# fhgyuanshen/HybridGL

Measured on AMD Instinct MI355X. Metric: images/sec (whole node), higher is better.
Workload: dtype f32 via fp16x3 split MFMA (fp32 accumulate)

## Files before the change

hybridgl_amd/_lib.py:

```python
import ctypes as C
import os

_HERE = os.path.dirname(os.path.abspath(__file__))
LIB_PATH = os.path.join(_HERE, "libhybridgl.so")

c_float_p = C.POINTER(C.c_float)
c_u8_p = C.POINTER(C.c_uint8)
c_i32_p = C.POINTER(C.c_int32)
c_i64_p = C.POINTER(C.c_int64)


class HybridGLError(RuntimeError):
    pass


class HglSentence(C.Structure):
    _fields_ = [("sentence_row", C.c_int), ("noun_phrase_row", C.c_int), ("other_row0", C.c_int), ("n_other", C.c_int),
                ("dirflag", C.c_int), ("relaword", C.c_int), ("has_other_nouns", C.c_int), ("black", C.c_float),
                ("imgattn", C.c_void_p), ("target", C.c_void_p)]


class HglGroupRef(C.Structure):
    _fields_ = [("hybrid", C.c_void_p), ("text", C.c_void_p), ("T", C.c_int), ("boxes", C.c_void_p), ("masks", C.c_void_p),
                ("N", C.c_int), ("H", C.c_int), ("W", C.c_int), ("sentences", C.POINTER(HglSentence)), ("S", C.c_int),
# ... 123 lines not shown
    "hgl_resize_bilinear_aa": (_I, [_VP, _I, _I, _I, _VP, _I, _I, _VP]),
    "hgl_resize_bilinear": (_I, [_VP, _I, _I, _I, _VP, _I, _I, _VP]),
    "hgl_mask_resize": (_I, [_VP, _I, _I, _I, _I, _VP, _VP]),
    "hgl_calculate_score": (_I, [_VP, _VP, _I, _I, _I, _F, _VP, _VP]),
    "hgl_coherence_workspace_bytes": (_SZ, [_I, _I, _I]),
    "hgl_coherence_scores": (_I, [_VP, _VP, _I, _I, _I, _I, _F, _VP, _VP, _SZ, _VP]),
    "hgl_iou": (_I, [_VP, _VP, _LL, _VP, _VP]),
    "hgl_iou_select": (_I, [_VP, _VP, _I, _VP, _LL, _VP, _VP]),
    "hgl_score_sentence_workspace_bytes": (_SZ, [_I, _I]),
    "hgl_score_sentence": (_I, [_VP, _VP, _VP, _VP, _I, _F, _VP, _VP, _I, _I, _F, _I, _I, _F, _I, _I,
                                _VP, _VP, _VP, _VP, _SZ, _VP]),
    "hgl_synthesize_views": (_I, [_VP, _VP, _VP, _VP, _I, _I, _I, _I, _VP, _VP, _VP]),
    "hgl_resize_pil_bilinear_workspace_bytes": (_SZ, [_I, _I, _I]),
    "hgl_resize_pil_bilinear": (_I, [_VP, _I, _I, _I, _I, _I, _VP, _VP, _I, _VP, _VP, _I, _VP, _VP, _SZ, _VP]),
    "hgl_sam_encode_workspace_bytes": (_SZ, [C.POINTER(HglSamEncoderW)]),
    "hgl_sam_encode": (_I, [C.POINTER(HglSamEncoderW), _VP, _I, _I, _VP, _VP, _SZ, _VP]),
    "hgl_sam_encode_batch_workspace_bytes": (_SZ, [C.POINTER(HglSamEncoderW), _I]),
    "hgl_sam_encode_batch": (_I, [C.POINTER(HglSamEncoderW), C.POINTER(C.c_void_p), C.POINTER(C.c_int), C.POINTER(C.c_int), _I,
                                  _VP, _VP, _SZ, _VP]),
    "hgl_sam_relpos_tables_workspace_bytes": (_SZ, [_I, _I, _I, _I]),
    "hgl_sam_relpos_tables": (_I, [_VP, _VP, _VP, _I, _I, _I, _I, _I, _I, _VP, _VP, _VP, _VP, _VP, _SZ, _VP]),
    "hgl_sam_dense_pe": (_I, [C.POINTER(HglSamDecoderW), _VP, _VP, _VP]),
    "hgl_sam_decode_workspace_bytes": (_SZ, [C.POINTER(HglSamDecoderW), _I]),
    "hgl_sam_decode_points": (_I, [C.POINTER(HglSamDecoderW), _VP, _VP, _I, _VP, _VP, _VP, _SZ, _VP]),
    "hgl_sam_decode_points_gated": (_I, [C.POINTER(HglSamDecoderW), _VP, _VP, _I, C.c_float, _VP, _VP, _VP, _SZ, _VP]),
    "hgl_sam_decode_multi_workspace_bytes": (_SZ, [C.POINTER(HglSamDecoderW), _I, _I]),
    "hgl_sam_decode_points_multi": (_I, [C.POINTER(HglSamDecoderW), _VP, _VP, _I, _I, _VP, _VP, _VP, _SZ, _VP]),
    "hgl_sam_decode_points_multi_gated": (_I, [C.POINTER(HglSamDecoderW), _VP, _VP, _I, _I, C.c_float, _VP, _VP, _VP, _SZ, _VP]),
    "hgl_sam_decode_prompts": (_I, [C.POINTER(HglSamDecoderW), _VP, _VP, _VP, _I, _VP, _I, _I, _VP, _VP, _VP, _SZ, _VP]),
    "hgl_sam_embed_masks": (_I, [C.POINTER(HglSamDecoderW), _VP, _I, _VP, _VP]),
    "hgl_sam_decoder_fusion": (_I, [_I]),
    "hgl_attention_presplit": (_I, [_I]),
    "hgl_attention_presplit_f32": (_I, [_VP, _I, _I, _I, _I, _I, _VP, _I, C.c_float, _I, _VP, _I, _I, _VP, C.c_size_t, _VP]),
    "hgl_sam_postprocess_workspace_bytes": (_SZ, [_I]),
    "hgl_sam_postprocess": (_I, [_VP, _VP, _I, _I, _I, _I, _I, _I, _I, _I, _F, _F, _F, _F, _VP, _VP, _VP, _VP, _VP,
                                 _VP, _SZ, _VP]),
    "hgl_nms": (_I, [_VP, _VP, _VP, _I, _F, _VP, _VP, _VP]),
    "hgl_nms_segments": (_I, [_VP, _VP, _VP, _VP, _I, _I, _F, _VP, _VP, _VP]),
    "hgl_nms_large_workspace_bytes": (_SZ, [_I]),
    "hgl_nms_large": (_I, [_VP, _VP, _VP, _I, _F, _VP, _VP, _VP, _SZ, _VP]),
    "hgl_box_near_crop_edge": (_I, [_VP, _I, C.POINTER(C.c_int32), C.POINTER(C.c_int32), _F, _VP, _VP]),
    "hgl_remove_small_regions_workspace_bytes": (_SZ, [_I, _I, _I]),
    "hgl_remove_small_regions": (_I, [_VP, _I, _I, _I, _I, _I, _VP, _VP, _VP, _SZ, _VP]),
    "hgl_remove_small_regions_boxes": (_I, [_VP, _I, _I, _I, _I, _I, _VP, _VP, _VP, _VP, _SZ, _VP]),
    "hgl_mask_boxes": (_I, [_VP, _I, _I, _I, _VP, _VP]),
    "hgl_gather_masks": (_I, [_VP, _VP, _VP, _I, _LL, _VP, _VP]),
    "hgl_gen_dir_mask": (_I, [_I, _I, _I, _VP, _VP]),
    "hgl_relation_boxes": (_I, [_VP, _VP, _VP, _VP, _I, _I, _VP, _VP]),
    "hgl_gaussian_blur_u8_workspace_bytes": (_SZ, [_I, _I, _I]),
    "hgl_gaussian_blur_u8": (_I, [_VP, _I, _I, _I, C.POINTER(C.c_double), _I, _VP, _VP, _SZ, _VP]),
    "hgl_cv_gaussian_kernel_q8": (_I, [_I, C.c_double, C.POINTER(C.c_uint16)]),
    "hgl_gaussian_blur_u8_q8": (_I, [_VP, _I, _I, _I, C.POINTER(C.c_uint16), C.POINTER(C.c_uint16), _I, _VP, _VP, _SZ, _VP]),
    "hgl_score_ref_workspace_bytes": (_SZ, [_I, _I, _I, _I, _I]),
    "hgl_score_ref": (_I, [_VP, _VP, _I, _VP, _VP, _I, _I, _I, _I, C.POINTER(HglSentence), _I, C.c_float, C.c_float, _I, _I, C.c_float,
                           _VP, _VP, _VP, _VP, _VP, _VP, _VP, _SZ, _VP]),
    "hgl_score_group_workspace_bytes": (_SZ, [C.POINTER(HglGroupRef), _I, _I]),
    "hgl_score_group": (_I, [C.POINTER(HglGroupRef), _I, _I, C.c_float, C.c_float, C.c_float, _VP, _VP, _SZ, _VP]),
    "hgl_score_group_sweep_workspace_bytes": (_SZ, [C.POINTER(HglGroupRef), _I, _I, C.POINTER(HglSweepConfig), _I]),
    "hgl_score_group_sweep": (_I, [C.POINTER(HglGroupRef), C.POINTER(HglSweepRef), _I, _I, C.c_float, C.POINTER(HglSweepConfig), _I,
                                   _VP, _VP, _VP, _SZ, _VP]),
    "hgl_u8_to_chw_lut": (_I, [_VP, _I, _I, _I, _VP, _VP, _VP]),
    "hgl_gt_mask_from_polygons": (_I, [_VP, _VP, _I, _I, _I, _VP, _VP]),
    "hgl_gt_mask_from_rle_counts": (_I, [_VP, _I, _I, _I, _VP, _VP]),
    "hgl_gt_mask_from_rle_string": (_I, [C.c_char_p, _I, _I, _VP, _VP]),
    "hgl_rle_encode_mask": (_I, [_VP, _I, _I, _VP, _LL, C.POINTER(C.c_longlong)]),
    "hgl_rle_to_string": (_I, [_VP, _LL, C.c_char_p, _SZ, C.POINTER(C.c_size_t)]),
# ... 56 lines not shown
```

hybridgl_amd/csrc/attention_ps.hip:

```cpp
#include "hgl_common.h"
#include "attn_tile.h"
#include <stdlib.h>
#include <mutex>
#include <type_traits>

namespace {

typedef __attribute__((address_space(3))) void lds_void_t;

constexpr int PS_CHUNK = 32;

enum { PS_PLAIN = 0, PS_WIN14 = 1, PS_RELT = 2 };

struct PsArgs {
  const _Float16 *hi, *lo;
  int ld, qcol, kcol, vcol;
  long long sb;
  int B, H, S;
  float* out;
  _Float16 *out_hi, *out_lo;
  int ldo;
  long long sob;
  float scale;
  int mask_kind;
  const uint8_t* keep;
  int keep_b0, keep_n;
  const float *rel_h, *rel_w;
  int kh, kw;
  const _Float16 *tabh_hi, *tabh_lo, *tabw_hi, *tabw_lo;
  int nqb;
  int dbg;
};
#ifdef HGL_DIAG
#define PS_DBG(a) ((a).dbg)
#else
#define PS_DBG(a) 0
#endif

__device__ __forceinline__ void ps_glds16(const void* sbase, unsigned voff, unsigned lds_addr) {
  unsigned keep;
  asm volatile("s_mov_b32 %0, m0\n\ts_mov_b32 m0, %3\n\ts_nop 0\n\tglobal_load_lds_dwordx4 %1, %2\n\ts_mov_b32 m0, %0"
               : "=&s"(keep)
               : "v"(voff), "s"(sbase), "s"(lds_addr)
               : "memory");
}
// ... 204 lines not shown
  const auto sw = __builtin_amdgcn_permlane32_swap(u, u, false, false);
  return fmaxf(__builtin_bit_cast(float, (unsigned)sw[0]), __builtin_bit_cast(float, (unsigned)sw[1]));
}
__device__ __forceinline__ float ps_add_halves(float x) {
  const unsigned u = __builtin_bit_cast(unsigned, x);
  const auto sw = __builtin_amdgcn_permlane32_swap(u, u, false, false);
  return __builtin_bit_cast(float, (unsigned)sw[0]) + __builtin_bit_cast(float, (unsigned)sw[1]);
}
template <int HD>
struct PspGeom {
  static constexpr int KS = HD / 16, DT = (HD + 31) / 32;
  static constexpr int KSL = HD / 4 + 1, KP = KSL * 8;
  static constexpr int VSL = 12, VP = VSL * 8;
  static constexpr int NIK = (PS_CHUNK * KSL + 63) / 64;
  static constexpr int NJK = (NIK + 3) / 4;
  static constexpr int KSTAGE = NIK * 1024;
  static constexpr int NIV = 2 * PS_CHUNK * VSL / 64;
  static constexpr int NJV = NIV / 4;
  static constexpr int VSTAGE = NIV * 1024;
  static constexpr int VL_OFF = PS_CHUNK * VSL * 16;
  static constexpr int K_RING = 0, V_RING = 3 * KSTAGE, E_OFF = V_RING + 2 * VSTAGE;
  static_assert(DT * 32 <= VP && NIV % 4 == 0, "geometry");
};
constexpr int PSP_EBYTES = PS_EROWS * 64;

template <int HD, int MODE>
constexpr size_t psp_lds_bytes() {
  return (size_t)PspGeom<HD>::E_OFF + (MODE == PS_WIN14 ? PSP_EBYTES : 0) + 256;
}

template <int HD, int MODE, int QT = 1>
__global__ __launch_bounds__(256, 2) void attn_psp_kernel(PsArgs a, const unsigned char* __restrict__ etab) {
  static_assert(QT == 1 || (QT == 2 && MODE == PS_PLAIN), "two query tiles per wave: the plain mode only");
  using G = PspGeom<HD>;
  constexpr int KS = G::KS, DT = G::DT, KP = G::KP, VP = G::VP;
  extern __shared__ __attribute__((aligned(1024))) unsigned char ps_smem[];
  uint8_t* const keepL = ps_smem + G::E_OFF + (MODE == PS_WIN14 ? PSP_EBYTES : 0);

  const int t = threadIdx.x, lane = t & 63;
  const int wave = __builtin_amdgcn_readfirstlane(t >> 6);
  const int r = lane & 31, h = lane >> 5;
  const float NEG_INF = __int_as_float(NEG_BIG_BITS);
  constexpr float LOG2E = 1.4426950408889634f;
  const float sl2e = a.scale * LOG2E;
  const float inv_scale = 1.0f / a.scale;
  const float rescale_thr = 5.5f * inv_scale;

  const unsigned ldb = (unsigned)a.ld * 2u;
  const unsigned lo_delta = (unsigned)((const char*)a.lo - (const char*)a.hi);
  const unsigned vrel = (unsigned)(a.vcol - a.kcol) * 2u;
  unsigned k_row[G::NJK], k_col[G::NJK], v_row[G::NJV], v_col[G::NJV];
#pragma unroll
  for (int j = 0; j < G::NJK; ++j) {
    const unsigned n = 64u * (unsigned)(wave + 4 * j) + (unsigned)lane;
    unsigned row = n / (unsigned)G::KSL;
    const unsigned c = n - row * (unsigned)G::KSL;
    unsigned col = 0;
    if (c < (unsigned)(HD / 8)) col = 16u * c;
    else if (c < (unsigned)(HD / 4)) col = 16u * (c - (unsigned)(HD / 8)) + lo_delta;
    if (row >= (unsigned)PS_CHUNK) row = 0;
    k_row[j] = row;
    k_col[j] = col;
  }
#pragma unroll
  for (int j = 0; j < G::NJV; ++j) {
    const unsigned n = 64u * (unsigned)(wave + 4 * j) + (unsigned)lane;
// ... 41 lines not shown
    if ((a.B & 7) == 0) {
      int be, rem;
      attn_xcd_item(L, (unsigned)a.H * nqb, be, rem);
      item = (int)((unsigned)be * (unsigned)a.H + (unsigned)rem / nqb);
      bx = (int)((unsigned)rem % nqb);
    } else {
      item = (int)(L / nqb);
      bx = (int)(L % nqb);
    }
  }
  const int b = item / a.H, hh = item - b * a.H;
  kv_base = (const char*)a.hi + ((long long)b * a.sb * (long long)a.ld + a.kcol + hh * HD) * 2;
  if (L != blockIdx.x) __syncthreads();
  if (!(PS_DBG(a) & 4)) {
  issue_k(0);
  issue_v(0);
  if (nchunk > 1) issue_k(1);
  }

  const uint8_t* keep_row = nullptr;
  if (MODE == PS_PLAIN && a.mask_kind == HGL_MASK_CLS_KEEP && b >= a.keep_b0)
    keep_row = a.keep + (long long)((b - a.keep_b0) % a.keep_n) * (a.S - 1);
  if (keep_row && t < a.S - 1) keepL[t] = keep_row[t];

  const int q0 = (bx * 4 + wave) * QT * 32;
  int qi[QT];
  bool qvalid[QT], tile_active[QT];
  h16x8 qh[QT][KS], ql[QT][KS];
#pragma unroll
  for (int qt = 0; qt < QT; ++qt) {
    qi[qt] = q0 + 32 * qt + r;
    qvalid[qt] = qi[qt] < a.S;
    tile_active[qt] = q0 + 32 * qt < a.S;
    const long long qo = ((long long)b * a.sb + (qvalid[qt] ? qi[qt] : 0)) * a.ld + a.qcol + hh * HD + 8 * h;
#pragma unroll
    for (int sx = 0; sx < KS; ++sx) {
      qh[qt][sx] = *(const h16x8*)(a.hi + qo + 16 * sx);
      ql[qt][sx] = *(const h16x8*)(a.lo + qo + 16 * sx);
    }
  }
  __builtin_amdgcn_sched_barrier(0);
#pragma unroll
  for (int qt = 0; qt < QT; ++qt) {
    if (!qvalid[qt]) {
#pragma unroll
      for (int sx = 0; sx < KS; ++sx)
#pragma unroll
        for (int e = 0; e < 8; ++e) { qh[qt][sx][e] = (_Float16)0.f; ql[qt][sx][e] = (_Float16)0.f; }
    }
  }
  const bool wave_active = tile_active[0];

  f32x16 o[QT][DT];
  float m_run[QT], l_run[QT];
#pragma unroll
  for (int qt = 0; qt < QT; ++qt) {
    m_run[qt] = NEG_INF;
    l_run[qt] = 0.f;
#pragma unroll
    for (int d = 0; d < DT; ++d)
#pragma unroll
      for (int e = 0; e < 16; ++e) o[qt][d][e] = 0.f;
  }

  h16x8 rbh[2], rbl[2];
  if constexpr (MODE == PS_WIN14) {
// ... 25 lines not shown
          acc = __builtin_amdgcn_mfma_f32_32x32x16_f16(tlr[sx], qh[0][sx], acc, 0, 0, 0);
          acc = __builtin_amdgcn_mfma_f32_32x32x16_f16(thr[sx], ql[0][sx], acc, 0, 0, 0);
          acc = __builtin_amdgcn_mfma_f32_32x32x16_f16(thr[sx], qh[0][sx], acc, 0, 0, 0);
        }
#pragma unroll
        for (int e = 0; e < 16; ++e) P0[((e & 3) + 8 * (e >> 2) + 4 * h) * 32 + r] = acc[e];
        __builtin_amdgcn_wave_barrier();
        __builtin_amdgcn_fence(__ATOMIC_RELEASE, "wavefront");
        const int qc = axis ? qx : qy;
#pragma unroll
        for (int c = 0; c < 2; ++c)
#pragma unroll
          for (int j = 0; j < 8; ++j) {
            const int k = 16 * c + 8 * h + j - 14 * axis;
            if (k >= 0 && k < 14) xs[c][j] = P0[(qc + 13 - k) * 32 + r];
          }
        __builtin_amdgcn_wave_barrier();
        __builtin_amdgcn_fence(__ATOMIC_ACQUIRE, "wavefront");
      }
    }
#pragma unroll
    for (int c = 0; c < 2; ++c)
#pragma unroll
      for (int j = 0; j < 8; ++j) {
        float x = xs[c][j] * inv_scale;
        _Float16 hi, lo;
        hgl_split_hi_lo(x, hi, lo);
        rbh[c][j] = hi;
        rbl[c][j] = lo;
      }
  }

  float rh_next = 0.f;
  f32x4 rw_next[4];
  auto rel_prefetch = [&](int kb) {
    if constexpr (MODE == PS_RELT) {
      int ln;
      asm volatile("v_mbcnt_lo_u32_b32 %0, -1, 0\n\tv_mbcnt_hi_u32_b32 %0, -1, %0" : "=v"(ln));
      const unsigned row = (unsigned)item * (unsigned)a.S + (unsigned)min(q0 + (ln & 31), a.S - 1);
      const unsigned relh_off = row * (unsigned)a.kh;
      const unsigned relw_off = row * (unsigned)a.kw + 4u * (unsigned)(ln >> 5);
      kb = min(kb, a.S - 32);
      rh_next = a.rel_h[relh_off + (unsigned)(kb / a.kw)];
      const unsigned o2 = relw_off + (unsigned)(kb % a.kw);
#pragma unroll
      for (int g4 = 0; g4 < 4; ++g4) rw_next[g4] = *(const f32x4*)(a.rel_w + o2 + 8 * g4);
    }
  };
  if (MODE == PS_RELT && wave_active) rel_prefetch(0);

  asm volatile("s_waitcnt vmcnt(0)" ::: "memory");
#pragma unroll
  for (int qt = 0; qt < QT; ++qt)
#pragma unroll
    for (int sx = 0; sx < KS; ++sx) asm volatile("" : "+v"(qh[qt][sx]), "+v"(ql[qt][sx]));
  if constexpr (MODE == PS_RELT) {
    asm volatile("" : "+v"(rh_next), "+v"(rw_next[0]), "+v"(rw_next[1]), "+v"(rw_next[2]), "+v"(rw_next[3]));
  }
  __syncthreads();

  auto qk = [&](int ci, f32x16& s, const h16x8 (&QH)[KS], const h16x8 (&QL)[KS]) {
    const _Float16* krow = (const _Float16*)(ps_smem + G::K_RING + (ci % 3) * G::KSTAGE) + k_off;
    attn_qk_tile<HD, 3>(krow, QH, QL, s);
    if constexpr (MODE == PS_WIN14) {
      const unsigned char* eb = ps_smem + G::E_OFF + ci * (PS_CHUNK * 64);
#pragma unroll
      for (int c = 0; c < 2; ++c) {
        const h16x8 e8 = *(const h16x8*)(eb + e_off[c]);
        s = __builtin_amdgcn_mfma_f32_32x32x16_f16(e8, rbl[c], s, 0, 0, 0);
        s = __builtin_amdgcn_mfma_f32_32x32x16_f16(e8, rbh[c], s, 0, 0, 0);
      }
    }
  };
  auto s_init = [&](f32x16& s) {
    if constexpr (MODE == PS_RELT) {
      const float rhs = rh_next * inv_scale;
#pragma unroll
      for (int e = 0; e < 16; ++e) s[e] = fmaf(rw_next[e >> 2][e & 3], inv_scale, rhs);
    } else {
#pragma unroll
      for (int e = 0; e < 16; ++e) s[e] = 0.f;
    }
  };

  f32x16 s_cur;
  if (wave_active) {
    s_init(s_cur);
    qk(0, s_cur, qh[0], ql[0]);
    if (MODE == PS_RELT && nchunk > 1) rel_prefetch(32);
  }

  for (int ci = 0; ci < nchunk; ++ci) {
    if (ci > 0) {
      asm volatile("s_waitcnt vmcnt(0)" ::: "memory");
      if constexpr (MODE == PS_RELT) {
        asm volatile("" : "+v"(rh_next), "+v"(rw_next[0]), "+v"(rw_next[1]), "+v"(rw_next[2]), "+v"(rw_next[3]));
      }
      __syncthreads();
    }
    if (!(PS_DBG(a) & 4)) {
    if (ci + 2 < nchunk) issue_k(ci + 2);
    if (ci + 1 < nchunk) issue_v(ci + 1);
    }
    if (!wave_active) continue;
    const int kbase = ci * PS_CHUNK;
    const bool has_next = ci + 1 < nchunk;
    auto tile = [&](auto cur_c, auto nxt_c, bool wn, int nci) {
      constexpr int CUR = decltype(cur_c)::value, NXT = decltype(nxt_c)::value;
      attn_mask_tail(s_cur, kbase, a.S, h);
      if (MODE == PS_PLAIN && CUR == 0 && keep_row && bx == 0 && wave == 0)
        attn_mask_cls_keep(s_cur, keepL, kbase, a.S, lane, h, qi[0]);
      f32x16 s_next;
      h16x8 ph[2], pl[2];
      float alpha = 1.0f;
      bool need;
      auto seg_a = [&](auto with_next) {
        constexpr bool WN = decltype(with_next)::value;
        constexpr int NM = WN ? 3 * KS + (MODE == PS_WIN14 ? 4 : 0) : 0;
        constexpr int NG = 19;
        const _Float16* krow = (const _Float16*)(ps_smem + G::K_RING + (nci % 3) * G::KSTAGE) + k_off;
        const unsigned char* eb = ps_smem + G::E_OFF + nci * (PS_CHUNK * 64);
        h16x8 fa, fb, fa2, fb2;
        if constexpr (WN) {
          s_init(s_next);
          fa = *(const h16x8*)(krow);
          fb = *(const h16x8*)(krow + HD);
        }
        auto mfma_i = [&](int i) {
          if constexpr (WN) {
            if (i < 3 * KS) {
              const int c = i / 3, term = i - 3 * c;
              if (term == 0) {
                if (c + 1 < KS) {
                  fa2 = *(const h16x8*)(krow + 16 * (c + 1));
                  fb2 = *(const h16x8*)(krow + HD + 16 * (c + 1));
                } else if (MODE == PS_WIN14) {
                  fa2 = *(const h16x8*)(eb + e_off[0]);
                  fb2 = *(const h16x8*)(eb + e_off[1]);
                }
                s_next = __builtin_amdgcn_mfma_f32_32x32x16_f16(fb, qh[NXT][c], s_next, 0, 0, 0);
              } else if (term == 1) {
                s_next = __builtin_amdgcn_mfma_f32_32x32x16_f16(fa, ql[NXT][c], s_next, 0, 0, 0);
              } else {
                s_next = __builtin_amdgcn_mfma_f32_32x32x16_f16(fa, qh[NXT][c], s_next, 0, 0, 0);
                fa = fa2;
                fb = fb2;
              }
            } else if (MODE == PS_WIN14) {
              const int j = i - 3 * KS;
              const h16x8 e8 = j < 2 ? fa : fb;
              s_next = __builtin_amdgcn_mfma_f32_32x32x16_f16(e8, (j & 1) ? rbh[j >> 1] : rbl[j >> 1], s_next, 0, 0, 0);
            }
          }
        };
        float mxa = NEG_INF, mxb = NEG_INF, m_use0 = 0.f, mneg = 0.f, rs = 0.f;
        float pe[16];
        h16x2 hi2[8];
// ... 25 lines not shown
                pe[2 * k + 1] = __builtin_amdgcn_exp2f(fmaf(s_cur[2 * k + 1], sl2e, mneg));
              }
              if (g == gf[k]) {
                rs += pe[2 * k];
                rs += pe[2 * k + 1];
                hi2[k] = __builtin_bit_cast(h16x2, __builtin_amdgcn_cvt_pkrtz(pe[2 * k], pe[2 * k + 1]));
              }
              if (g == gg[k]) {
                const int e = 2 * k;
                ph[e >> 3][e & 7] = hi2[k][0]; ph[e >> 3][(e & 7) + 1] = hi2[k][1];
                pl[e >> 3][e & 7] = (_Float16)(pe[e] - (float)hi2[k][0]);
                pl[e >> 3][(e & 7) + 1] = (_Float16)(pe[e + 1] - (float)hi2[k][1]);
              }
            }
          }
        };
#pragma unroll
        for (int g = 0; g < NG; ++g) {
#pragma unroll
          for (int i = g * NM / NG; i < (g + 1) * NM / NG; ++i) mfma_i(i);
          valu_g(g);
          __builtin_amdgcn_sched_barrier(0);
        }
        l_run[CUR] += rs;
      };
      if (wn) seg_a(std::true_type());
      else seg_a(std::false_type());
      if (need) {
#pragma unroll
        for (int d = 0; d < DT; ++d)
#pragma unroll
          for (int e = 0; e < 16; ++e) o[CUR][d][e] *= alpha;
      }
      if (MODE == PS_RELT && ci + 2 < nchunk) rel_prefetch(kbase + 64);
      if (!(PS_DBG(a) & 2)) {
        const _Float16* Vh = (const _Float16*)(ps_smem + G::V_RING + (ci & 1) * G::VSTAGE);
        const _Float16* Vl = (const _Float16*)(ps_smem + G::V_RING + (ci & 1) * G::VSTAGE + G::VL_OFF);
        attn_pv_tile<DT, VP, 3>(Vh, Vl, tr_off, kbase, a.S, ph, pl, o[CUR]);
      }
      if (wn) s_cur = s_next;
    };
    using I0 = std::integral_constant<int, 0>;
    using I1 = std::integral_constant<int, QT - 1>;
    const bool chain = !(PS_DBG(a) & 1);
    if constexpr (QT == 2) {
      tile(I0(), I1(), true, ci);
      tile(I1(), I0(), has_next, ci + 1);
    } else {
      tile(I0(), I0(), has_next && chain, ci + 1);
    }
  }

#pragma unroll
  for (int qt = 0; qt < QT; ++qt) {
  const float l_tot = ps_add_halves(l_run[qt]);
  const float inv = l_tot > 0.f ? 1.0f / l_tot : 0.f;
  if (tile_active[qt] && !(PS_DBG(a) & 8)) {
    const long long orow = b * a.sob + (long long)(qvalid[qt] ? qi[qt] : 0) * a.ldo + hh * HD;
#pragma unroll
    for (int d = 0; d < DT; ++d)
#pragma unroll
      for (int g = 0; g < 4; g += 2) {
        if (d * 32 + 8 * g >= HD) continue;
        f32x4 w0, w1;
#pragma unroll
        for (int e = 0; e < 4; ++e) { w0[e] = o[qt][d][4 * g + e] * inv; w1[e] = o[qt][d][4 * (g + 1) + e] * inv; }
        if (a.out) {
          if (qvalid[qt]) {
            *(f32x4*)(a.out + orow + d * 32 + 8 * g + 4 * h) = w0;
            *(f32x4*)(a.out + orow + d * 32 + 8 * (g + 1) + 4 * h) = w1;
          }
        } else {
          h16x4 hi0, lo0, hi1, lo1;
#pragma unroll
          for (int e = 0; e < 4; ++e) {
            _Float16 a2, c2;
            hgl_split_hi_lo(w0[e], a2, c2);
            hi0[e] = a2; lo0[e] = c2;
            hgl_split_hi_lo(w1[e], a2, c2);
            hi1[e] = a2; lo1[e] = c2;
          }
          typedef unsigned u32x2 __attribute__((ext_vector_type(2)));
          typedef unsigned u32x4s __attribute__((ext_vector_type(4)));
// ... 124 lines not shown
}

int hgl_launch_attention_planes(const HglAttn& d, HglAttnRoute route, hipStream_t st) {
  const int S = d.Sq;
  HGL_REQUIRE(d.qkv_hi && d.qkv_lo && (d.out || (d.out_hi && d.out_lo)) && d.B > 0 && d.H > 0 && S > 0, "attention_ps: bad arguments");
  HGL_REQUIRE((d.ld & 7) == 0 && (d.qcol & 7) == 0 && (d.kcol & 7) == 0 && (d.vcol & 7) == 0 && (d.ldo & 3) == 0 && (d.sob & 3) == 0 &&
                  (((uintptr_t)d.qkv_hi | (uintptr_t)d.qkv_lo | (uintptr_t)d.out | (uintptr_t)d.out_hi | (uintptr_t)d.out_lo) & 15) == 0,
              "attention_ps: operands must be 16-byte aligned");
  HGL_REQUIRE(d.mask_kind != HGL_MASK_CLS_KEEP || d.keep, "attention_ps: HGL_MASK_CLS_KEEP needs keep bytes");
  HGL_REQUIRE(d.vcol >= d.kcol, "attention_ps: the V columns must not lie before the K columns (32-bit offsets from the K base)");
  HGL_REQUIRE((d.rel_h == nullptr) == (d.rel_w == nullptr) && (d.tab_h == nullptr) == (d.tab_w == nullptr), "attention_ps: rel-pos operands go in pairs");
  PsArgs a;
  a.hi = (const _Float16*)d.qkv_hi; a.lo = (const _Float16*)d.qkv_lo;
  a.ld = d.ld; a.qcol = d.qcol; a.kcol = d.kcol; a.vcol = d.vcol; a.sb = d.sb;
  a.B = d.B; a.H = d.H; a.S = S;
  a.out = d.out; a.out_hi = (_Float16*)d.out_hi; a.out_lo = (_Float16*)d.out_lo; a.ldo = d.ldo; a.sob = d.sob;
  a.scale = d.scale; a.mask_kind = d.mask_kind; a.keep = d.keep; a.keep_b0 = d.keep_b0; a.keep_n = d.keep_n > 0 ? d.keep_n : d.B;
  a.rel_h = d.rel_h; a.rel_w = d.rel_w; a.kh = d.kh; a.kw = d.kw;
  a.tabh_hi = a.tabh_lo = a.tabw_hi = a.tabw_lo = nullptr;
  a.nqb = 1;
  a.dbg = HGL_DIAG_SWITCH("HGL_ATTN_PS_DBG", 0);
  if (route == HGL_ATTN_PS_WIN) {
    const void* t[4];
    (void)hgl_attention_rel_tables(d.tab_h, d.tab_w, t);
    a.tabh_hi = (const _Float16*)t[0]; a.tabh_lo = (const _Float16*)t[1];
    a.tabw_hi = (const _Float16*)t[2]; a.tabw_lo = (const _Float16*)t[3];
    a.nqb = 2;
  } else if (route != HGL_ATTN_PS_CLIP) {
    a.nqb = (S + 127) / 128;
  }
  HglProfScope prof(HGL_PROF_ATTN, 4.0 * d.B * d.H * (double)S * S * d.hd, 0.0, st);
  switch (route) {
    case HGL_ATTN_PS_WIN: return psp_launch<80, PS_WIN14>(a, st);
    case HGL_ATTN_PS_RELT: return d.hd == 80 ? psp_launch<80, PS_RELT>(a, st) : psp_launch<64, PS_RELT>(a, st);
    case HGL_ATTN_PS_PLAIN: return d.hd == 80 ? psp_launch<80, PS_PLAIN>(a, st) : psp_launch<64, PS_PLAIN>(a, st);
    default: return ps_launch<64, PS_PLAIN, 2>(a, st);
  }
}

extern "C" int hgl_attention_presplit_f32(const float* qkv, int ld, int B, int H, int S, int hd, float* out, int ldo, float scale,
                                          int mask_kind, const uint8_t* keep, int keep_b0, int keep_n, void* scratch,
                                          size_t scratch_bytes, void* stream) {
  HGL_TRY(hgl_require_device());
  HGL_REQUIRE(qkv && out && scratch && B > 0 && H > 0 && S > 0 && ld >= 3 * H * hd && (ld & 7) == 0, "attention_presplit: bad arguments");
  const size_t n = (size_t)B * S * ld;
  HGL_REQUIRE(scratch_bytes >= n * 4, "attention_presplit: scratch too small (%zu bytes for %zu)", scratch_bytes, n * 4);
  HGL_REQUIRE(hgl_split_layout() && hgl_split_terms() == 3, "attention_presplit: f16x3 mode only");
  hipStream_t st = (hipStream_t)stream;
  uint16_t* hi = (uint16_t*)scratch;
  uint16_t* lo = hi + n;
  HGL_TRY(hgl_launch_split_f16(qkv, 1.0f, hi, lo, (long long)n, st));
  HglAttn d = hgl_attn_packed_planes(hi, lo, B, H, S, hd);
  d.ld = ld, d.scale = scale;
  d.out = out, d.ldo = ldo, d.sob = (long long)S * ldo;
  d.mask_kind = mask_kind, d.keep = keep, d.keep_b0 = keep_b0, d.keep_n = keep_n;
  const int prev = hgl_attention_presplit(1);
  const bool served = hgl_attention_route(d) != HGL_ATTN_NONE;
  const int rc = served ? hgl_launch_attention(d, st) : HGL_OK;
  hgl_attention_presplit(prev);
  HGL_REQUIRE(served, "attention_presplit: shape not served (B %d, H %d, S %d, hd %d, mask %d)", B, H, S, hd, mask_kind);
  return rc;
}
```

hybridgl_amd/ops.py:

```python
import ctypes as C
from itertools import repeat

import torch

from . import _lib
from ._lib import check

ACT = {"none": 0, "quickgelu": 1, "gelu": 2, "relu": 3}
MASK = {"none": 0, "causal": 1, "cls_keep": 2}
DIRFLAG = {"none": 0, "left": 1, "right": 2, "middle": 3}
RELAWORD = {"none": 0, "left": 1, "right": 2, "up": 3, "down": 4, "big": 5, "small": 6, "within": 7}


def _stream():
    return torch.cuda.current_stream().cuda_stream


def _dev(t, dtype, name):
    if not isinstance(t, torch.Tensor):
        raise TypeError(f"{name}: expected a torch.Tensor")
    if not t.is_cuda:
        raise _lib.HybridGLError(f"{name}: tensor must live on the GPU (no CPU path exists)")
    if t.dtype != dtype:
        raise TypeError(f"{name}: expected dtype {dtype}, got {t.dtype}")
# ... 180 lines not shown
    y = torch.empty_like(x)
    check(lib.hgl_layernorm_f32(_dev(x, torch.float32, "x"), _dev(w, torch.float32, "w"),
                                _dev(b, torch.float32, "b"), _dev(y, torch.float32, "y"), rows, D,
                                float(eps), _stream()), "hgl_layernorm_f32")
    return y


def attention(q, k, v, heads, scale=None, mask="none", keep=None, keep_b0=0, keep_n=0,
              rel_h=None, rel_w=None):
    lib = _lib.load()
    B, Sq, Dm = q.shape
    Sk = k.shape[1]
    hd = Dm // heads
    if scale is None:
        scale = hd ** -0.5
    out = torch.empty_like(q)
    kp = None
    if keep is not None:
        kp, keep = _u8(keep, "keep")
    kh = kw = 0
    if rel_h is not None:
        kh, kw = rel_h.shape[-1], rel_w.shape[-1]
    check(lib.hgl_attention_f32(_dev(q, torch.float32, "q"), _dev(k, torch.float32, "k"),
                                _dev(v, torch.float32, "v"), _dev(out, torch.float32, "out"),
                                B, heads, Sq, Sk, hd, Dm, Dm, Dm, Dm,
                                Sq * Dm, Sk * Dm, Sk * Dm, Sq * Dm, float(scale), MASK[mask], kp,
                                keep_b0, keep_n,
                                _dev(rel_h, torch.float32, "rel_h") if rel_h is not None else None,
                                _dev(rel_w, torch.float32, "rel_w") if rel_w is not None else None,
                                kh, kw, _stream()), "hgl_attention_f32")
    return out


def attention_presplit(qkv, heads, scale=None, mask="none", keep=None, keep_b0=0, keep_n=0):
    lib = _lib.load()
    B, S, D3 = qkv.shape
    Dm = D3 // 3
    hd = Dm // heads
    if scale is None:
        scale = hd ** -0.5
    out = torch.empty((B, S, Dm), dtype=torch.float32, device=qkv.device)
    scratch = torch.empty(B * S * D3, dtype=torch.float32, device=qkv.device)
    kp = None
    if keep is not None:
        kp, keep = _u8(keep, "keep")
    check(lib.hgl_attention_presplit_f32(_dev(qkv, torch.float32, "qkv"), D3, B, heads, S, hd, _dev(out, torch.float32, "out"), Dm,
                                         float(scale), MASK[mask], kp, keep_b0, keep_n, scratch.data_ptr(), scratch.numel() * 4,
                                         _stream()), "hgl_attention_presplit_f32")
    return out


def sam_relpos_tables(q, rel_pos_h, rel_pos_w, B, heads, size, rel_h=None, rel_w=None):
    lib = _lib.load()
    S = size * size
    hd = rel_pos_h.shape[1]
    planes = isinstance(q, (tuple, list))
    q0 = q[0] if planes else q
    assert q0.shape[0] == B * S and tuple(rel_pos_h.shape) == tuple(rel_pos_w.shape) == (2 * size - 1, hd)
    if rel_h is None:
        rel_h = torch.empty((B * heads, S, size), dtype=torch.float32, device=q0.device)
    if rel_w is None:
        rel_w = torch.empty((B * heads, S, size), dtype=torch.float32, device=q0.device)
    assert tuple(rel_h.shape) == tuple(rel_w.shape) == (B * heads, S, size)
    need = lib.hgl_sam_relpos_tables_workspace_bytes(B, heads, S, size)
    ws = workspace(need, q0.device, "sam_relpos")
    check(lib.hgl_sam_relpos_tables(None if planes else _dev(q, torch.float32, "q"),
                                    _dev(q[0], torch.float16, "q_hi") if planes else None,
                                    _dev(q[1], torch.float16, "q_lo") if planes else None, q0.shape[1], B, heads, S, size, hd,
                                    _dev(rel_pos_h, torch.float32, "rel_pos_h"), _dev(rel_pos_w, torch.float32, "rel_pos_w"),
                                    _dev(rel_h, torch.float32, "rel_h"), _dev(rel_w, torch.float32, "rel_w"), ws.data_ptr(), need,
                                    _stream()), "hgl_sam_relpos_tables")
    return rel_h, rel_w


def mask_resize(masks, g):
    lib = _lib.load()
    N, H, W = masks.shape
    mp, masks = _u8(masks, "masks")
# ... 800 lines not shown
```

include/hybridgl.h:

```cpp
#ifndef HYBRIDGL_H
#define HYBRIDGL_H

#include <stddef.h>
#include <stdint.h>

#ifdef __cplusplus
extern "C" {
#endif

#define HGL_OK 0
#define HGL_EINVAL (-1)
#define HGL_ENODEVICE (-2)
#define HGL_EWORKSPACE (-3)
#define HGL_ELAUNCH (-4)

#define HGL_ABI_VERSION 7

#define HGL_ACT_NONE 0
#define HGL_ACT_QUICKGELU 1
#define HGL_ACT_GELU 2
#define HGL_ACT_RELU 3

#define HGL_FUSION_G2L 0
#define HGL_FUSION_L2G 1
// ... 263 lines not shown
int hgl_sam_encode_batch(const HglSamEncoderW* w, const uint8_t* const* resized_imgs, const int* in_h, const int* in_w,
                         int nb, float* emb, void* workspace, size_t workspace_bytes, void* stream);

size_t hgl_sam_relpos_tables_workspace_bytes(int B, int heads, int S, int size);
int hgl_sam_relpos_tables(const float* qkv, const void* q_hi, const void* q_lo, int ldq, int B, int heads, int S, int size,
                          int hd, const float* rel_pos_h, const float* rel_pos_w, float* rel_h, float* rel_w,
                          void* workspace, size_t workspace_bytes, void* stream);

int hgl_sam_dense_pe(const HglSamDecoderW* w, const float* grid_coords01, float* dense_pe, void* stream);

size_t hgl_sam_decode_workspace_bytes(const HglSamDecoderW* w, int P);
int hgl_sam_decode_points(const HglSamDecoderW* w, const float* emb, const float* points01, int P,
                          float* low_res, float* iou_pred, void* workspace, size_t workspace_bytes,
                          void* stream);
int hgl_sam_decode_points_gated(const HglSamDecoderW* w, const float* emb, const float* points01, int P, float iou_gate,
                                float* low_res, float* iou_pred, void* workspace, size_t workspace_bytes, void* stream);
size_t hgl_sam_decode_multi_workspace_bytes(const HglSamDecoderW* w, int n_img, int ppi);
int hgl_sam_decode_points_multi(const HglSamDecoderW* w, const float* emb, const float* points01, int n_img, int ppi,
                                float* low_res, float* iou_pred, void* workspace, size_t workspace_bytes, void* stream);
int hgl_sam_decode_points_multi_gated(const HglSamDecoderW* w, const float* emb, const float* points01, int n_img, int ppi,
                                      float iou_gate, float* low_res, float* iou_pred, void* workspace, size_t workspace_bytes,
                                      void* stream);
int hgl_sam_decode_prompts(const HglSamDecoderW* w, const float* emb, const float* coords01, const int32_t* labels, int n_sparse,
                           const float* dense, int first_mask, int P, float* low_res, float* iou_pred, void* workspace,
                           size_t workspace_bytes, void* stream);
int hgl_sam_embed_masks(const HglSamDecoderW* w, const float* mask_input, int P, float* dense, void* stream);

int hgl_sam_decoder_fusion(int mask);

int hgl_attention_presplit(int on);
int hgl_attention_presplit_f32(const float* qkv, int ld, int B, int H, int S, int hd, float* out, int ldo, float scale,
                               int mask_kind, const uint8_t* keep, int keep_b0, int keep_n, void* scratch,
                               size_t scratch_bytes, void* stream);

size_t hgl_sam_postprocess_workspace_bytes(int K);
int hgl_sam_postprocess(const float* low_res, const float* iou_pred, int K, int hl, int wl, int img_size,
                        int in_h, int in_w, int H, int W, float mask_threshold, float stability_offset,
                        float pred_iou_thresh, float stability_thresh, uint8_t* masks, int32_t* boxes_xyxy,
                        float* stability, uint8_t* keep, float* full_logits, void* workspace,
                        size_t workspace_bytes, void* stream);

int hgl_nms(const int32_t* boxes_xyxy, const float* scores, const uint8_t* keep, int K, float iou_threshold,
            int32_t* out_idx, int32_t* out_n, void* stream);

int hgl_nms_segments(const int32_t* boxes_xyxy, const float* scores, const uint8_t* keep, const int32_t* offsets, int n_seg,
                     int max_len, float iou_threshold, int32_t* out_idx, int32_t* out_n, void* stream);

size_t hgl_remove_small_regions_workspace_bytes(int N, int H, int W);
int hgl_remove_small_regions(const uint8_t* masks, int N, int H, int W, int area_thresh, int holes,
                             uint8_t* out, uint8_t* changed, void* workspace, size_t workspace_bytes,
                             void* stream);
int hgl_remove_small_regions_boxes(const uint8_t* masks, int N, int H, int W, int area_thresh, int holes,
                                   uint8_t* out, uint8_t* changed, int32_t* boxes_xyxy, void* workspace,
                                   size_t workspace_bytes, void* stream);
size_t hgl_nms_large_workspace_bytes(int K);
int hgl_nms_large(const int32_t* boxes_xyxy, const float* scores, const uint8_t* keep, int K, float iou_threshold,
                  int32_t* out_idx, int32_t* out_n, void* workspace, size_t workspace_bytes, void* stream);
int hgl_box_near_crop_edge(const int32_t* boxes_xyxy, int K, const int32_t* crop_box_xyxy, const int32_t* orig_box_xyxy,
                           float atol, uint8_t* keep, void* stream);
int hgl_mask_boxes(const uint8_t* masks, int N, int H, int W, int32_t* boxes_xyxy, void* stream);

int hgl_gather_masks(const uint8_t* masks, const int32_t* idx, const int32_t* n, int max_n, long long HW,
                     uint8_t* out, void* stream);

int hgl_gt_mask_from_polygons(const double* xy, const int32_t* n_points, int n_polys, int H, int W, uint8_t* mask,
                              int64_t* area);
// ... 63 lines not shown
```

Before: 34.51.

## Load rel-pos width terms once per query row when kw is 64

Adds a specialised path of the presplit attention kernel for relative-position attention whose width is 64. Each lane loads its whole 64-wide rel_w row into registers once, and the chunk loop is unrolled by two so each chunk picks the matching half. This replaces the per-chunk rel_w prefetch, leaving only the scalar rel_h term to fetch per chunk. It costs extra registers, and the general chunked variant is kept for other widths. A new C/Python entry point for rel-pos presplit attention and some diagnostic switches are also added.

```diff
diff --git a/hybridgl_amd/_lib.py b/hybridgl_amd/_lib.py
--- a/hybridgl_amd/_lib.py
+++ b/hybridgl_amd/_lib.py
@@ -179,6 +179,7 @@
     "hgl_sam_decoder_fusion": (_I, [_I]),
     "hgl_attention_presplit": (_I, [_I]),
     "hgl_attention_presplit_f32": (_I, [_VP, _I, _I, _I, _I, _I, _VP, _I, C.c_float, _I, _VP, _I, _I, _VP, C.c_size_t, _VP]),
+    "hgl_attention_presplit_rel_f32": (_I, [_VP, _I, _I, _I, _I, _I, _VP, _I, C.c_float, _VP, _VP, _I, _I, _VP, C.c_size_t, _VP]),
     "hgl_sam_postprocess_workspace_bytes": (_SZ, [_I]),
     "hgl_sam_postprocess": (_I, [_VP, _VP, _I, _I, _I, _I, _I, _I, _I, _I, _F, _F, _F, _F, _VP, _VP, _VP, _VP, _VP,
                                  _VP, _SZ, _VP]),
diff --git a/hybridgl_amd/csrc/attention_ps.hip b/hybridgl_amd/csrc/attention_ps.hip
--- a/hybridgl_amd/csrc/attention_ps.hip
+++ b/hybridgl_amd/csrc/attention_ps.hip
@@ -10,7 +10,7 @@
 
 constexpr int PS_CHUNK = 32;
 
-enum { PS_PLAIN = 0, PS_WIN14 = 1, PS_RELT = 2 };
+enum { PS_PLAIN = 0, PS_WIN14 = 1, PS_RELT = 2, PS_RELT_CHUNK = 3 };
 
 struct PsArgs {
   const _Float16 *hi, *lo;
@@ -281,6 +281,8 @@
 template <int HD, int MODE, int QT = 1>
 __global__ __launch_bounds__(256, 2) void attn_psp_kernel(PsArgs a, const unsigned char* __restrict__ etab) {
   static_assert(QT == 1 || (QT == 2 && MODE == PS_PLAIN), "two query tiles per wave: the plain mode only");
+  constexpr bool RELT = MODE == PS_RELT || MODE == PS_RELT_CHUNK;
+  constexpr bool RW64 = MODE == PS_RELT;
   using G = PspGeom<HD>;
   constexpr int KS = G::KS, DT = G::DT, KP = G::KP, VP = G::VP;
   extern __shared__ __attribute__((aligned(1024))) unsigned char ps_smem[];
@@ -388,6 +390,9 @@
     qi[qt] = q0 + 32 * qt + r;
     qvalid[qt] = qi[qt] < a.S;
     tile_active[qt] = q0 + 32 * qt < a.S;
+#ifdef HGL_DIAG
+    if (MODE == PS_WIN14 && (PS_DBG(a) & 64) && b % 25 >= 20 && q0 + 32 * qt >= 112) tile_active[qt] = false;
+#endif
     const long long qo = ((long long)b * a.sb + (qvalid[qt] ? qi[qt] : 0)) * a.ld + a.qcol + hh * HD + 8 * h;
 #pragma unroll
     for (int sx = 0; sx < KS; ++sx) {
@@ -479,29 +484,54 @@
   }
 
   float rh_next = 0.f;
-  f32x4 rw_next[4];
+  f32x4 rw_next[RW64 ? 1 : 4];
+  f32x4 rw_all[RW64 ? 2 : 1][4];
+#ifdef HGL_DIAG
+  if (PS_DBG(a) & 32)
+    for (auto& x : rw_next) x = f32x4{0.f, 0.f, 0.f, 0.f};
+#endif
   auto rel_prefetch = [&](int kb) {
-    if constexpr (MODE == PS_RELT) {
+    if constexpr (RELT) {
       int ln;
       asm volatile("v_mbcnt_lo_u32_b32 %0, -1, 0\n\tv_mbcnt_hi_u32_b32 %0, -1, %0" : "=v"(ln));
       const unsigned row = (unsigned)item * (unsigned)a.S + (unsigned)min(q0 + (ln & 31), a.S - 1);
       const unsigned relh_off = row * (unsigned)a.kh;
-      const unsigned relw_off = row * (unsigned)a.kw + 4u * (unsigned)(ln >> 5);
-      kb = min(kb, a.S - 32);
-      rh_next = a.rel_h[relh_off + (unsigned)(kb / a.kw)];
-      const unsigned o2 = relw_off + (unsigned)(kb % a.kw);
-#pragma unroll
-      for (int g4 = 0; g4 < 4; ++g4) rw_next[g4] = *(const f32x4*)(a.rel_w + o2 + 8 * g4);
+      if constexpr (RW64) {
+        rh_next = a.rel_h[relh_off + ((unsigned)kb >> 6)];
+      } else {
+        const unsigned relw_off = row * (unsigned)a.kw + 4u * (unsigned)(ln >> 5);
+        kb = min(kb, a.S - 32);
+        rh_next = a.rel_h[relh_off + (unsigned)(kb / a.kw)];
+        const unsigned o2 = relw_off + (unsigned)(kb % a.kw);
+        if (!(PS_DBG(a) & 32)) {
+#pragma unroll
+        for (int g4 = 0; g4 < 4; ++g4) rw_next[g4] = *(const f32x4*)(a.rel_w + o2 + 8 * g4);
+        }
+      }
     }
   };
-  if (MODE == PS_RELT && wave_active) rel_prefetch(0);
+  if constexpr (RW64) {
+    if (wave_active) {
+      const unsigned row = (unsigned)item * (unsigned)a.S + (unsigned)min(q0 + r, a.S - 1);
+      const float* const rw = a.rel_w + row * 64u + 4u * (unsigned)h;
+#pragma unroll
+      for (int p = 0; p < 2; ++p)
+#pragma unroll
+        for (int g4 = 0; g4 < 4; ++g4) rw_all[p][g4] = *(const f32x4*)(rw + 32 * p + 8 * g4);
+    }
+  }
+  if (RELT && wave_active) rel_prefetch(0);
 
   asm volatile("s_waitcnt vmcnt(0)" ::: "memory");
 #pragma unroll
   for (int qt = 0; qt < QT; ++qt)
 #pragma unroll
     for (int sx = 0; sx < KS; ++sx) asm volatile("" : "+v"(qh[qt][sx]), "+v"(ql[qt][sx]));
-  if constexpr (MODE == PS_RELT) {
+  if constexpr (RW64) {
+    asm volatile("" : "+v"(rh_next));
+#pragma unroll
+    for (int p = 0; p < 2; ++p) asm volatile("" : "+v"(rw_all[p][0]), "+v"(rw_all[p][1]), "+v"(rw_all[p][2]), "+v"(rw_all[p][3]));
+  } else if constexpr (RELT) {
     asm volatile("" : "+v"(rh_next), "+v"(rw_next[0]), "+v"(rw_next[1]), "+v"(rw_next[2]), "+v"(rw_next[3]));
   }
   __syncthreads();
@@ -519,8 +549,12 @@
       }
     }
   };
-  auto s_init = [&](f32x16& s) {
-    if constexpr (MODE == PS_RELT) {
+  auto s_init = [&](f32x16& s, int ph) {
+    if constexpr (RW64) {
+      const float rhs = rh_next * inv_scale;
+#pragma unroll
+      for (int e = 0; e < 16; ++e) s[e] = fmaf(rw_all[ph][e >> 2][e & 3], inv_scale, rhs);
+    } else if constexpr (RELT) {
       const float rhs = rh_next * inv_scale;
 #pragma unroll
       for (int e = 0; e < 16; ++e) s[e] = fmaf(rw_next[e >> 2][e & 3], inv_scale, rhs);
@@ -532,15 +566,23 @@
 
   f32x16 s_cur;
   if (wave_active) {
-    s_init(s_cur);
+    s_init(s_cur, 0);
     qk(0, s_cur, qh[0], ql[0]);
-    if (MODE == PS_RELT && nchunk > 1) rel_prefetch(32);
-  }
-
-  for (int ci = 0; ci < nchunk; ++ci) {
-    if (ci > 0) {
+    if (RELT && nchunk > 1) rel_prefetch(32);
+  }
+
+  constexpr int CU = RW64 ? 2 : 1;
+  for (int ci0 = 0; ci0 < nchunk; ci0 += CU) {
+  int ci = ci0;
+#pragma unroll
+  do {
+    if constexpr (RW64) {
       asm volatile("s_waitcnt vmcnt(0)" ::: "memory");
-      if constexpr (MODE == PS_RELT) {
+      asm volatile("" : "+v"(rh_next));
+      if (ci > 0) __syncthreads();
+    } else if (ci > 0) {
+      asm volatile("s_waitcnt vmcnt(0)" ::: "memory");
+      if constexpr (RELT) {
         asm volatile("" : "+v"(rh_next), "+v"(rw_next[0]), "+v"(rw_next[1]), "+v"(rw_next[2]), "+v"(rw_next[3]));
       }
       __syncthreads();
@@ -569,7 +611,7 @@
         const unsigned char* eb = ps_smem + G::E_OFF + nci * (PS_CHUNK * 64);
         h16x8 fa, fb, fa2, fb2;
         if constexpr (WN) {
-          s_init(s_next);
+          s_init(s_next, (nci - ci0) & 1);
           fa = *(const h16x8*)(krow);
           fb = *(const h16x8*)(krow + HD);
         }
@@ -661,7 +703,7 @@
 #pragma unroll
           for (int e = 0; e < 16; ++e) o[CUR][d][e] *= alpha;
       }
-      if (MODE == PS_RELT && ci + 2 < nchunk) rel_prefetch(kbase + 64);
+      if (RELT && ci + 2 < nchunk) rel_prefetch(kbase + 64);
       if (!(PS_DBG(a) & 2)) {
         const _Float16* Vh = (const _Float16*)(ps_smem + G::V_RING + (ci & 1) * G::VSTAGE);
         const _Float16* Vl = (const _Float16*)(ps_smem + G::V_RING + (ci & 1) * G::VSTAGE + G::VL_OFF);
@@ -678,6 +720,7 @@
     } else {
       tile(I0(), I0(), has_next && chain, ci + 1);
     }
+  } while (RW64 && ++ci < ci0 + CU);
   }
 
 #pragma unroll
@@ -868,15 +911,19 @@
   HglProfScope prof(HGL_PROF_ATTN, 4.0 * d.B * d.H * (double)S * S * d.hd, 0.0, st);
   switch (route) {
     case HGL_ATTN_PS_WIN: return psp_launch<80, PS_WIN14>(a, st);
-    case HGL_ATTN_PS_RELT: return d.hd == 80 ? psp_launch<80, PS_RELT>(a, st) : psp_launch<64, PS_RELT>(a, st);
+    case HGL_ATTN_PS_RELT: {
+      static const int rw64_on = HGL_DIAG_SWITCH("HGL_ATTN_PS_RW64", 1);
+      if (d.kw == 64 && rw64_on) return d.hd == 80 ? psp_launch<80, PS_RELT>(a, st) : psp_launch<64, PS_RELT>(a, st);
+      return d.hd == 80 ? psp_launch<80, PS_RELT_CHUNK>(a, st) : psp_launch<64, PS_RELT_CHUNK>(a, st);
+    }
     case HGL_ATTN_PS_PLAIN: return d.hd == 80 ? psp_launch<80, PS_PLAIN>(a, st) : psp_launch<64, PS_PLAIN>(a, st);
     default: return ps_launch<64, PS_PLAIN, 2>(a, st);
   }
 }
 
-extern "C" int hgl_attention_presplit_f32(const float* qkv, int ld, int B, int H, int S, int hd, float* out, int ldo, float scale,
-                                          int mask_kind, const uint8_t* keep, int keep_b0, int keep_n, void* scratch,
-                                          size_t scratch_bytes, void* stream) {
+static int attention_presplit_f32(const float* qkv, int ld, int B, int H, int S, int hd, float* out, int ldo, float scale, int mask_kind,
+                                  const uint8_t* keep, int keep_b0, int keep_n, const float* rel_h, const float* rel_w, int kh, int kw,
+                                  void* scratch, size_t scratch_bytes, void* stream) {
   HGL_TRY(hgl_require_device());
   HGL_REQUIRE(qkv && out && scratch && B > 0 && H > 0 && S > 0 && ld >= 3 * H * hd && (ld & 7) == 0, "attention_presplit: bad arguments");
   const size_t n = (size_t)B * S * ld;
@@ -890,10 +937,25 @@
   d.ld = ld, d.scale = scale;
   d.out = out, d.ldo = ldo, d.sob = (long long)S * ldo;
   d.mask_kind = mask_kind, d.keep = keep, d.keep_b0 = keep_b0, d.keep_n = keep_n;
+  d.rel_h = rel_h, d.rel_w = rel_w, d.kh = rel_h ? kh : 0, d.kw = rel_h ? kw : 0;
   const int prev = hgl_attention_presplit(1);
   const bool served = hgl_attention_route(d) != HGL_ATTN_NONE;
   const int rc = served ? hgl_launch_attention(d, st) : HGL_OK;
   hgl_attention_presplit(prev);
-  HGL_REQUIRE(served, "attention_presplit: shape not served (B %d, H %d, S %d, hd %d, mask %d)", B, H, S, hd, mask_kind);
+  HGL_REQUIRE(served, "attention_presplit: shape not served (B %d, H %d, S %d, hd %d, mask %d, rel-pos %d x %d)", B, H, S, hd, mask_kind,
+              d.kh, d.kw);
   return rc;
 }
+extern "C" int hgl_attention_presplit_f32(const float* qkv, int ld, int B, int H, int S, int hd, float* out, int ldo, float scale,
+                                          int mask_kind, const uint8_t* keep, int keep_b0, int keep_n, void* scratch,
+                                          size_t scratch_bytes, void* stream) {
+  return attention_presplit_f32(qkv, ld, B, H, S, hd, out, ldo, scale, mask_kind, keep, keep_b0, keep_n, nullptr, nullptr, 0, 0, scratch,
+                                scratch_bytes, stream);
+}
+extern "C" int hgl_attention_presplit_rel_f32(const float* qkv, int ld, int B, int H, int S, int hd, float* out, int ldo, float scale,
+                                              const float* rel_h, const float* rel_w, int kh, int kw, void* scratch,
+                                              size_t scratch_bytes, void* stream) {
+  HGL_REQUIRE(rel_h && rel_w && kh > 0 && kw > 0, "attention_presplit_rel: the rel-pos terms are required");
+  return attention_presplit_f32(qkv, ld, B, H, S, hd, out, ldo, scale, HGL_MASK_NONE, nullptr, 0, 0, rel_h, rel_w, kh, kw, scratch,
+                                scratch_bytes, stream);
+}
diff --git a/hybridgl_amd/ops.py b/hybridgl_amd/ops.py
--- a/hybridgl_amd/ops.py
+++ b/hybridgl_amd/ops.py
@@ -236,7 +236,7 @@
     return out
 
 
-def attention_presplit(qkv, heads, scale=None, mask="none", keep=None, keep_b0=0, keep_n=0):
+def attention_presplit(qkv, heads, scale=None, mask="none", keep=None, keep_b0=0, keep_n=0, rel_h=None, rel_w=None):
     lib = _lib.load()
     B, S, D3 = qkv.shape
     Dm = D3 // 3
@@ -248,6 +248,15 @@
     kp = None
     if keep is not None:
         kp, keep = _u8(keep, "keep")
+    if rel_h is not None:
+        if mask != "none" or rel_w is None:
+            raise ValueError("attention_presplit: rel-pos terms go in pairs and take no mask")
+        check(lib.hgl_attention_presplit_rel_f32(_dev(qkv, torch.float32, "qkv"), D3, B, heads, S, hd, _dev(out, torch.float32, "out"),
+                                                 Dm, float(scale), _dev(rel_h, torch.float32, "rel_h"),
+                                                 _dev(rel_w, torch.float32, "rel_w"), rel_h.shape[-1], rel_w.shape[-1],
+                                                 scratch.data_ptr(), scratch.numel() * 4, _stream()),
+              "hgl_attention_presplit_rel_f32")
+        return out
     check(lib.hgl_attention_presplit_f32(_dev(qkv, torch.float32, "qkv"), D3, B, heads, S, hd, _dev(out, torch.float32, "out"), Dm,
                                          float(scale), MASK[mask], kp, keep_b0, keep_n, scratch.data_ptr(), scratch.numel() * 4,
                                          _stream()), "hgl_attention_presplit_f32")
diff --git a/include/hybridgl.h b/include/hybridgl.h
--- a/include/hybridgl.h
+++ b/include/hybridgl.h
@@ -319,6 +319,9 @@
 int hgl_attention_presplit_f32(const float* qkv, int ld, int B, int H, int S, int hd, float* out, int ldo, float scale,
                                int mask_kind, const uint8_t* keep, int keep_b0, int keep_n, void* scratch,
                                size_t scratch_bytes, void* stream);
+int hgl_attention_presplit_rel_f32(const float* qkv, int ld, int B, int H, int S, int hd, float* out, int ldo, float scale,
+                                   const float* rel_h, const float* rel_w, int kh, int kw, void* scratch,
+                                   size_t scratch_bytes, void* stream);
 
 size_t hgl_sam_postprocess_workspace_bytes(int K);
 int hgl_sam_postprocess(const float* low_res, const float* iou_pred, int K, int hl, int wl, int img_size,
```

Result: no change. 34.70, median of 6 (+0.6%).
